# grantneale/kafka-lag-based-assignor

Hardware: AMD Instinct MI355X
Metric: partition-assignments/sec (whole node) (higher is better)
Workload: dtype int64

## Files before the change

kafka_lag_based_assignor_amd/csrc/la_api.hip:

```cpp
#include "la_ctx.h"

#include <dlfcn.h>

namespace {

constexpr int kMaxShards = 64;

struct HintSpender {
    la_ctx* ctx;
    explicit HintSpender(la_ctx* c) : ctx(c) {}
    ~HintSpender() { if (ctx) ctx->hints_set = false; }
    HintSpender(const HintSpender&) = delete;
    HintSpender& operator=(const HintSpender&) = delete;
};

struct RcclApi {
    void* handle = nullptr;
    int (*CommInitAll)(void** comms, int ndev, const int* devlist) = nullptr;
    int (*CommDestroy)(void* comm) = nullptr;
    int (*AllGather)(const void* send, void* recv, size_t count, int datatype, void* comm, hipStream_t stream) = nullptr;
    int (*GroupStart)() = nullptr;
    int (*GroupEnd)() = nullptr;
    const char* (*GetErrorString)(int) = nullptr;
    std::string why;
// ... 237 lines not shown
        g.out_pid = b->d_out_partition;
        g.out_rank = b->d_out_member_rank;
        g.out_total = b->d_out_total_lag;
        g.reset_latest = (b->reset_mode == LA_RESET_LATEST) ? 1 : 0;
        g.no_sample_sort = (b->flags & LA_FLAG_NO_SAMPLE_SORT) ? 1 : ((b->flags & LA_FLAG_SAMPLE_TIGHT) ? 2 : 0);
        g.sort_multi_kernel = (b->flags & LA_FLAG_SORT_MULTIKERNEL) ? 1 : 0;
        g.no_run_merge = (b->flags & LA_FLAG_NO_RUN_MERGE) ? 1 : 0;
        g.no_moved_sort = (b->flags & LA_FLAG_NO_MOVED_SORT) ? 1 : 0;
        const bool bounded_large = (b->flags & LA_FLAG_BOUNDS) && b->max_lag_hint >= 0 && b->max_partition_id_hint >= 0;
        g.max_lag_hint = bounded_large ? b->max_lag_hint : -1;
        g.max_id_hint = bounded_large ? b->max_partition_id_hint : -1;
        g.status = status;
        hipError_t e = hipSuccess;
        if (c > la::kLargeMaxConsumers) {
            if (int rc = flush()) return rc;
            if (argmin)
                return fail(ctx, LA_ESHAPE, "topic %lld has %lld consumers; LA_ALGO_ARGMIN (a test hook) holds at most %lld",
                            (long long)t, (long long)c, (long long)la::kLargeMaxConsumers);
            e = la::huge_topic_launch(ln.large, g, stream);
        } else if (argmin || p == 0 || (b->flags & LA_FLAG_SERIAL_LARGE)) {
            if (int rc = flush()) return rc;
            e = la::large_topic_launch(ln.large, g, argmin, stream);
        } else {
            if (group.size() >= kGroupTopics || (group_n > 0 && group_n + p > kGroupPartitions))
                if (int rc = flush()) return rc;
            group.push_back(g);
            group_n += p;
        }
        if (e != hipSuccess) return hip_fail(ctx, e, "large topic %lld: %s", (long long)t);
    }
    return flush();
}

}

int enqueue_batch(la_ctx* ctx, Lane& ln, const la_device_batch* b, hipStream_t stream, StagedBatch* staged) {
    uint32_t* const status = staged && staged->status ? staged->status : ln.d_status;
    const la::TileTail* const tail = staged ? staged->tail : nullptr;
    bool* const tail_done = staged ? &staged->tail_done : nullptr;
    if (b->n_topics < 0 || b->n_partitions < 0 || b->n_consumers < 0)
        return fail(ctx, LA_EINVAL, "negative size");
    if (b->n_topics == 0) return LA_OK;
    if (!b->d_part_off || !b->d_cons_off) return fail(ctx, LA_EINVAL, "null offsets");
    const bool wire_out = (b->flags & LA_FLAG_WIRE_OUT) != 0;
    if (b->n_partitions > 0 && !wire_out && (!b->d_out_partition || !b->d_out_member_rank)) return fail(ctx, LA_EINVAL, "null outputs");
    if (wire_out) {
        if (!b->d_out_wire || (b->wire_elem_bytes != 2 && b->wire_elem_bytes != 4) ||
            !la::wire_format_valid(b->wire_elem_bytes, b->wire_id_bits))
            return fail(ctx, LA_EINVAL, "LA_FLAG_WIRE_OUT: d_out_wire and a 2- or 4-byte wire format are required");
        if (b->algo != LA_ALGO_AUTO || (b->flags & LA_FLAG_RAGGED) ||
            !la::wave_tile_fits(b->max_partitions_per_topic, b->max_consumers_per_topic) || b->n_partitions >= ((int64_t)1 << 29) ||
            b->n_consumers >= ((int64_t)1 << 30) || (b->flags & LA_FLAG_INDEX64) || !(b->flags & LA_FLAG_BOUNDS) ||
            !la::wave_tile_always_packs(b->max_partitions_per_topic, b->max_consumers_per_topic, b->max_lag_hint,
                                        b->max_partition_id_hint))
            return fail(ctx, LA_EINVAL, "LA_FLAG_WIRE_OUT needs a batch of tile-sized topics (shape hint within 1024 x 64, no LA_FLAG_RAGGED), "
                                        "LA_FLAG_BOUNDS that prove every tile packs, and fewer than 2^29 partitions: run this batch "
                                        "without the flag and pack the results with la_pack_results_on");
    }
    if (b->n_partitions > 0 && (!b->d_partition_id || (!b->d_lag && (!b->d_end_off || !b->d_committed_off))))
        return fail(ctx, LA_EINVAL, "null per-partition input");
    if (b->n_consumers > 0 && !b->d_cons_rank) return fail(ctx, LA_EINVAL, "null cons_rank");
    if (!b->d_lag && b->reset_mode != LA_RESET_LATEST && !b->d_begin_off && b->n_partitions > 0)
        return fail(ctx, LA_EINVAL, "begin_off is required unless reset_mode is LA_RESET_LATEST");
    if (b->algo != LA_ALGO_AUTO && b->algo != LA_ALGO_ROUNDS && b->algo != LA_ALGO_ARGMIN && b->algo != LA_ALGO_ROUNDS_WIDE)
        return fail(ctx, LA_EINVAL, "unknown algo %d", b->algo);

    la::TileArgs a{};
    a.n_topics = b->n_topics;
    a.part_off = b->d_part_off;
    a.pid = b->d_partition_id;
    a.begin = b->d_begin_off;
    a.end = b->d_end_off;
    a.committed = b->d_committed_off;
    a.lag = b->d_lag;
    a.cons_off = b->d_cons_off;
    a.cons_rank = b->d_cons_rank;
    a.out_pid = b->d_out_partition;
    a.out_rank = b->d_out_member_rank;
    a.out_total = b->d_out_total_lag;
    a.status = status;
    a.reset_latest = (b->reset_mode == LA_RESET_LATEST) ? 1 : 0;
    a.n_total = b->n_partitions;
    a.flags = b->flags & (LA_FLAG_INDEX64 | LA_FLAG_DEFER_WIDE);
    if (getenv("LA_TILE_ALWAYS_STAGE2")) a.flags |= la::kTileAlwaysStage2;
    if (wire_out) {
        a.flags |= la::kTileWireOut;
        a.out_wire = b->d_out_wire;
        a.wire_bytes = b->wire_elem_bytes;
        a.wire_id_bits = b->wire_id_bits;
    }
    a.topic_list = nullptr;
    a.k_total = b->n_consumers;
    if (int rc = reserve(ctx, ln.defer, la::wave_tile_defer_bytes(b->n_topics))) return rc;
    a.defer_list = (int32_t*)ln.defer.p;
    const bool argmin = (b->algo == LA_ALGO_ARGMIN);
    const int tile_mode = argmin ? 2 : (b->algo == LA_ALGO_ROUNDS_WIDE ? 1 : 0);

    hipStreamCaptureStatus capture = hipStreamCaptureStatusNone;
    if (tile_mode == 0) LA_HIP(ctx, hipStreamIsCapturing(stream, &capture));
    hipError_t counter_err = hipSuccess;
    const bool bounded = tile_mode == 0 && (b->flags & LA_FLAG_BOUNDS) && b->max_lag_hint >= 0 && b->max_partition_id_hint >= 0;
    auto proven = [&](int64_t mp, int64_t mc) {
        return bounded && la::wave_tile_always_packs(mp, mc, b->max_lag_hint, b->max_partition_id_hint);
    };
    auto next_counters = [&](la::TileArgs& t) {
        int32_t* pair = (int32_t*)(ln.d_status + 16);
        if (t.flags & la::kTileNoDefer) {
            t.defer_count = pair + (ln.launches & 1u);
            t.defer_count_next = pair + ((ln.launches + 1u) & 1u);
            return;
        }
        if (capture != hipStreamCaptureStatusNone) {
            t.defer_count = pair + 2;
            t.defer_count_next = pair + 3;
            const hipError_t e = hipMemsetAsync(pair + 2, 0, sizeof(int32_t), stream);
            if (e != hipSuccess) counter_err = e;
            return;
        }
        t.defer_count = pair + (ln.launches & 1u);
        t.defer_count_next = pair + ((ln.launches + 1u) & 1u);
        if (tile_mode == 0) ++ln.launches;
    };
    if (b->n_partitions == 0) {
        if (b->d_out_total_lag && b->n_consumers > 0)
            LA_HIP(ctx, hipMemsetAsync(b->d_out_total_lag, 0, (size_t)b->n_consumers * sizeof(int64_t), stream));
        return LA_OK;
    }
    ln.large.prof.armed = (b->flags & LA_FLAG_PROFILE) != 0;
    if (ln.large.prof.armed) ln.large.prof.recorded = false;
    const bool have_host = b->h_part_off && b->h_cons_off;
    const bool fits_hint = la::wave_tile_fits(b->max_partitions_per_topic, b->max_consumers_per_topic);
    if (fits_hint && !(have_host && (b->flags & LA_FLAG_RAGGED) && tile_mode == 0)) {
        if (proven(b->max_partitions_per_topic, b->max_consumers_per_topic)) a.flags |= la::kTileNoDefer;
        next_counters(a);
        LA_HIP(ctx, counter_err);
        if (tail && tile_mode == 0) a.tail = *tail;
        LA_HIP(ctx, la::wave_tile_launch(a, b->max_partitions_per_topic, b->max_consumers_per_topic, tile_mode, stream,
                                         tail_done));
        return LA_OK;
    }
    la_device_batch with_host;
    if (!have_host) {
        hipStreamCaptureStatus cap = hipStreamCaptureStatusNone;
        LA_HIP(ctx, hipStreamIsCapturing(stream, &cap));
        if (cap != hipStreamCaptureStatusNone)
            return fail(ctx, LA_EINVAL, "shape hint exceeds one wave tile: h_part_off and h_cons_off are required "
                                        "while the stream is being captured");
        const size_t words = (size_t)b->n_topics + 1;
        ln.host_offsets.resize(2 * words);
        LA_HIP(ctx, hipMemcpyAsync(ln.host_offsets.data(), b->d_part_off, words * 8, hipMemcpyDeviceToHost, stream));
        LA_HIP(ctx, hipMemcpyAsync(ln.host_offsets.data() + words, b->d_cons_off, words * 8, hipMemcpyDeviceToHost, stream));
        LA_HIP(ctx, hipStreamSynchronize(stream));
        with_host = *b;
        with_host.h_part_off = ln.host_offsets.data();
        with_host.h_cons_off = ln.host_offsets.data() + words;
        b = &with_host;
    }

    const bool use_block = !argmin && b->algo != LA_ALGO_ROUNDS_WIDE;
    BatchPlan plan;
    if (int rc = plan_batch(ctx, ln, b, tile_mode, use_block, &plan)) return rc;
    const int32_t* d_lists = nullptr;
    if (int rc = stage_topic_lists(ctx, ln, plan, b->n_topics, stream, &d_lists)) return rc;
    if (plan.classed) {
        for (int k = 0; k < kTileClasses; ++k) {
            if (plan.tile[k].n == 0) continue;
            la::TileArgs run = a;
// ... 1443 lines not shown
```

kafka_lag_based_assignor_amd/csrc/la_kernels.h:

```cpp
#pragma once
#include <hip/hip_runtime.h>
#include <stdint.h>

#include "la_launch.h"

namespace la {

constexpr uint32_t kStatusShape = 1u;
constexpr uint32_t kStatusUnsorted = 2u;
constexpr uint32_t kStatusInternal = 4u;

constexpr uint32_t kStatusOrder = 8u;

constexpr uint32_t kStatusWire = 16u;

constexpr uint32_t kStatusSparse = 32u;

constexpr uint32_t kStatusBounds = 64u;

constexpr uint32_t kStatusLoads = 128u;

constexpr uint32_t kStatusMoves = 256u;

constexpr uint32_t kStatusCoop = 2 * kStatusMoves;

constexpr uint32_t kStatusSticky = 2 * kStatusCoop;

constexpr uint32_t kStatusBits[] = {kStatusShape, kStatusUnsorted, kStatusInternal, kStatusOrder,  kStatusWire,  kStatusSparse,
                                    kStatusBounds, kStatusLoads,   kStatusMoves,    kStatusCoop,   kStatusSticky};
constexpr bool status_bits_distinct() {
    uint32_t seen = 0;
    for (uint32_t b : kStatusBits) {
        if (b == 0 || (b & (b - 1)) != 0 || (seen & b) != 0) return false;
        seen |= b;
    }
    return true;
}
static_assert(status_bits_distinct(), "every status bit is one bit of its own");

constexpr int32_t kTileNoDefer = 8;
constexpr int32_t kTileWireOut = 16;
constexpr int32_t kTileSkipOversize = 4;
constexpr int32_t kTileAlwaysStage2 = 32;

constexpr int64_t kTileMaxPartitions = 1024;
constexpr int64_t kTileMaxConsumers = 64;
constexpr int64_t kLargeMaxConsumers = 8192;

struct TileTail {
    int32_t enabled;
    int32_t n_members;
    int32_t n;
    int32_t pad_;
    int64_t n_topics;
    const int64_t* part_off;
    const int32_t* out_pid;
    const int32_t* out_rank;
    int64_t* member_off;
    int32_t* grouped_topic;
    int32_t* grouped_partition;
    uint32_t* counter;
    uint32_t* fin_flag;
};

struct TileArgs {
    int64_t n_topics;
    int64_t n_total;
    int64_t k_total;
    const int64_t* part_off;
    const int32_t* pid;
    const int64_t* begin;
    const int64_t* end;
    const int64_t* committed;
    const int64_t* lag;
    const int64_t* cons_off;
    const int32_t* cons_rank;
    int32_t* out_pid;
    int32_t* out_rank;
    int64_t* out_total;
    uint32_t* status;
    int32_t reset_latest;
    int32_t flags;
    const int32_t* topic_list;
    int32_t* defer_count;
    int32_t* defer_count_next;
    int32_t* defer_list;
    TileTail tail;
    void* out_wire;
    int32_t wire_bytes, wire_id_bits;
};

inline size_t wave_tile_defer_bytes(int64_t n_topics) { return (size_t)(n_topics > 0 ? n_topics : 1) * sizeof(int32_t); }

inline bool wave_tile_fits(int64_t max_p, int64_t max_c) {
    return max_p <= kTileMaxPartitions && max_c <= kTileMaxConsumers;
}
void wave_tile_pick(int64_t max_p, int64_t max_c, int* L, int* E);
bool wave_tile_always_packs(int64_t max_p, int64_t max_c, int64_t max_lag, int64_t max_id);
hipError_t wave_tile_launch(TileArgs a, int64_t max_p, int64_t max_c, int mode, hipStream_t stream, bool* tail_done = nullptr);

hipError_t lag_launch(int64_t n, const int64_t* begin, const int64_t* end, const int64_t* committed,
                      bool reset_latest, int64_t* out_lag, hipStream_t stream);

hipError_t sparse_begin_launch(int64_t m, const int64_t* idx, const int64_t* val, int64_t base, int64_t lo, int64_t hi,
                               int64_t* begin, uint32_t* status, hipStream_t stream);

hipError_t finish_status_launch(const uint32_t* d_status, uint32_t* h_flag, hipStream_t stream);
hipError_t wake_launch(hipStream_t stream);

hipError_t check_consumers_launch(int64_t n_topics, const int64_t* cons_off, const int32_t* cons_rank,
                                  uint32_t* status, hipStream_t stream);

constexpr int64_t kBlockMaxPartitions = 8192;
constexpr int64_t kBlockMaxConsumers = 2048;
constexpr int64_t kBlockWidePartitions = 16384;
constexpr int64_t kBlockWideConsumers = 1024;
constexpr int kBlockClasses = 5;

struct BlockArgs {
    const int64_t* part_off;
    const int64_t* cons_off;
    const int32_t* list;
    int32_t n_list;
    int32_t inline_list[8];
    const int32_t* pid;
    const int64_t* begin;
    const int64_t* end;
    const int64_t* committed;
    const int64_t* lag;
    const int32_t* cons_rank;
    int32_t* out_pid;
    int32_t* out_rank;
    int64_t* out_total;
    uint32_t* status;
    int32_t reset_latest;
    int32_t np_cap, nc_cap;
    int32_t dense_ids;
    int32_t key32_greedy;
    int32_t radix_sort;
};

inline bool block_fits(int64_t p, int64_t c) {
    return (p <= kBlockMaxPartitions && c <= kBlockMaxConsumers) || (p <= kBlockWidePartitions && c <= kBlockWideConsumers);
}
inline int block_class(int64_t p, int64_t c) {
    if (p <= 512 && c <= 256) return 0;
    if (p <= 2048 && c <= 256) return 1;
    if (p <= 4096 && c <= 1024) return 2;
    if (p <= kBlockMaxPartitions) return 3;
    return 4;
}
hipError_t block_launch(BlockArgs a, int cls, hipStream_t stream);

struct LargeProfile {
    hipEvent_t ev[4] = {};
    bool armed = false;
    bool recorded = false;
    int64_t n = 0;
};

struct LargeScratch {
    void* buf = nullptr;
    size_t cap = 0;
    LargeProfile prof;
    struct Stage {
        void* h = nullptr;
        size_t cap = 0;
        hipEvent_t done = nullptr;
    } stage[2];
    unsigned stage_next = 0;
    void* d_items = nullptr;
    size_t d_items_cap = 0;
};

// ... 175 lines not shown
```

kafka_lag_based_assignor_amd/csrc/la_wave_tile_impl.h:

```cpp
#pragma once
#include "la_kernels.h"
#include "la_device.h"
#include "la_sort64.h"
#include "la_sort32.h"
#include "la_group_small.h"
#ifdef LA_LAB
#include <cstdio>
#include <cstdlib>
#endif

namespace la {

enum : int { kModeAuto = 0, kModeWide = 1, kModeArgmin = 2 };

#ifndef LA_ABLATE
#define LA_ABLATE 0
#endif
constexpr int kAblate = LA_ABLATE;
#ifndef LA_SKIP_SORTED_ROUNDS
#define LA_SKIP_SORTED_ROUNDS 1
#endif
constexpr bool kSkipSortedRounds = LA_SKIP_SORTED_ROUNDS != 0;
#ifndef LA_WPB
#define LA_WPB 4
#endif

template <int L, int E>
struct TileCfg {
    static constexpr int kGroupsPerWave = kWave / L;
    static constexpr int kWavesPerBlock = LA_WPB;
    static constexpr int kThreads = kWave * kWavesPerBlock;
    static constexpr int kTopicsPerBlock = kGroupsPerWave * kWavesPerBlock;
    static constexpr int kCap = L * E;
    static constexpr int kSlots = kCap + (kCap >> 3) + 1;
    static constexpr int kLog2Cap = (kCap <= 1) ? 0 : (31 - __builtin_clz(kCap - 1)) + 1;
};

__device__ __forceinline__ int slot_of(int s) { return s + (s >> 3); }

struct __attribute__((aligned(8))) I64x2 { int64_t x, y; };
struct __attribute__((aligned(4))) I32x2 { int32_t x, y; };

template <int L, int E>
__device__ __forceinline__ int load_index(int v, int gl) {
    if constexpr (E >= 2) return (v >> 1) * (2 * L) + 2 * gl + (v & 1);
    else return gl;
}

template <int E>
struct Raw {
    I64x2 en[(E + 1) / 2];
    I64x2 cm[(E + 1) / 2];
    I32x2 id[(E + 1) / 2];
};

template <typename IDX>
struct TopicDescT {
    IDX p0, c0;
    int P, C;
};
using TopicDesc = TopicDescT<int64_t>;

#ifndef LA_NT_LOADS
#define LA_NT_LOADS 1
#endif
template <typename V, typename T, typename IDX>
__device__ __forceinline__ V load_at(const T* base, IDX idx) {
    const V* p;
    if constexpr (sizeof(IDX) == 4)
        p = reinterpret_cast<const V*>(reinterpret_cast<const char*>(base) + (uint32_t)(idx * (uint32_t)sizeof(T)));
    else
        p = reinterpret_cast<const V*>(base + idx);
#if LA_NT_LOADS
    if constexpr (sizeof(V) == 16) {
        typedef long long LL2 __attribute__((ext_vector_type(2), aligned(8)));
        const LL2 v = __builtin_nontemporal_load(reinterpret_cast<const LL2*>(p));
        V out;
        __builtin_memcpy(&out, &v, 16);
        return out;
    } else if constexpr (sizeof(V) == 8) {
        typedef int I2 __attribute__((ext_vector_type(2), aligned(4)));
        const I2 v = __builtin_nontemporal_load(reinterpret_cast<const I2*>(p));
        V out;
        __builtin_memcpy(&out, &v, 8);
        return out;
    } else {
        return *p;
    }
#else
    return *p;
#endif
}

template <int L, int E, bool FULL = false, typename D>
__device__ __forceinline__ auto clamped_index(const TileArgs& a, const D& d, int v, int gl) {
    using IDX = decltype(d.p0);
    const IDX g = d.p0 + (IDX)load_index<L, E>(v, gl);
    if constexpr (FULL) return g;
    const IDX hi = (IDX)(a.n_total - (E >= 2 ? 2 : 1));
    return g < hi ? g : hi;
}

template <int L, int E, bool FULL = false, typename D>
__device__ __forceinline__ void issue_loads(const TileArgs& a, const D& d, int gl, Raw<E>& raw) {
    if constexpr (kAblate == 2) return;
    constexpr int NP = (E + 1) / 2;
    const int64_t* src_en = a.lag ? a.lag : a.end;
    if (!a.lag) {
#pragma unroll
        for (int k = 0; k < NP; ++k) {
            const auto g = clamped_index<L, E, FULL>(a, d, 2 * k, gl);
            if constexpr (E >= 2) raw.cm[k] = load_at<I64x2>(a.committed, g);
            else { raw.cm[k].x = load_at<int64_t>(a.committed, g); raw.cm[k].y = 0; }
        }
    } else {
#pragma unroll
        for (int k = 0; k < NP; ++k) raw.cm[k].x = raw.cm[k].y = 0;
    }
#pragma unroll
    for (int k = 0; k < NP; ++k) {
        const auto g = clamped_index<L, E, FULL>(a, d, 2 * k, gl);
        if constexpr (E >= 2) {
            raw.en[k] = load_at<I64x2>(src_en, g);
            raw.id[k] = load_at<I32x2>(a.pid, g);
        } else {
            raw.en[k].x = load_at<int64_t>(src_en, g); raw.en[k].y = 0;
            raw.id[k].x = load_at<int32_t>(a.pid, g); raw.id[k].y = 0;
        }
    }
}

template <int L, int E>
__device__ __forceinline__ bool second_stage_needed(const TileArgs& a) {
    return !a.lag && !a.reset_latest && a.begin;
}

template <int L, int E, bool FULL = false, typename D>
__device__ __forceinline__ void issue_begin_loads(const TileArgs& a, const D& d, int gl, Raw<E>& raw) {
    if constexpr (kAblate == 2) return;
    constexpr int NP = (E + 1) / 2;
    if (!second_stage_needed<L, E>(a)) return;
    {
        bool any = false;
#pragma unroll
        for (int k = 0; k < NP; ++k) any |= (raw.cm[k].x < 0) | (E >= 2 && raw.cm[k].y < 0);
        if (__builtin_amdgcn_ballot_w64(any) == 0 && !(a.flags & kTileAlwaysStage2)) return;
    }
#pragma unroll
    for (int k = 0; k < NP; ++k) {
        const auto g = clamped_index<L, E, FULL>(a, d, 2 * k, gl);
        using G = decltype(g);
        const bool nx = raw.cm[k].x < 0;
        if constexpr (E >= 2) {
            const bool ny = raw.cm[k].y < 0;
            const I64x2 bv = load_at<I64x2>(a.begin, (nx | ny) ? g : (G)0);
            raw.cm[k].x = nx ? bv.x : raw.cm[k].x;
            raw.cm[k].y = ny ? bv.y : raw.cm[k].y;
        } else {
            const int64_t vx = a.begin[nx ? g : (G)0];
            raw.cm[k].x = nx ? vx : raw.cm[k].x;
        }
    }
}

template <int L, int E, bool FULL = false, typename D>
__device__ __forceinline__ void finish_lags(const TileArgs& a, const D& d, int gl, const Raw<E>& raw,
                                            int64_t (&lag)[E], int32_t (&pid)[E]) {
    const bool latest = a.reset_latest != 0;
    if constexpr (kAblate == 2) {
#pragma unroll
        for (int v = 0; v < E; ++v) {
            const uint32_t h = ((uint32_t)d.p0 + (uint32_t)(v * L + gl)) * 2654435761u;
            lag[v] = (int64_t)(h >> 2) + a.reset_latest;
            pid[v] = (int32_t)((v * L + gl) * 77 + 13) & (L * E - 1);
        }
        return;
    }
    constexpr int NP = (E + 1) / 2;
    const bool cm_is_next = second_stage_needed<L, E>(a);
    auto lag_of = [&](int64_t en, int64_t cm) -> int64_t {
        if (a.lag) return en;
        if (cm_is_next) { const int64_t dlt = (int64_t)((uint64_t)en - (uint64_t)cm); return dlt > 0 ? dlt : 0; }
        return partition_lag(0, en, cm, latest);
    };
#pragma unroll
    for (int k = 0; k < NP; ++k) {
        const int e = load_index<L, E>(2 * k, gl);
        const bool shifted = !FULL && (E >= 2) && (d.p0 + (decltype(d.p0))e == (decltype(d.p0))(a.n_total - 1));
        const int64_t en_x = shifted ? raw.en[k].y : raw.en[k].x;
        const int64_t cm_x = shifted ? raw.cm[k].y : raw.cm[k].x;
        pid[2 * k] = shifted ? raw.id[k].y : raw.id[k].x;
        lag[2 * k] = lag_of(en_x, cm_x);
        if constexpr (E >= 2) {
            pid[2 * k + 1] = raw.id[k].y;
            lag[2 * k + 1] = lag_of(raw.en[k].y, raw.cm[k].y);
        }
    }
    if constexpr (FULL) return;
#pragma unroll
    for (int v = 0; v < E; ++v) {
        const bool valid = load_index<L, E>(v, gl) < d.P;
        lag[v] = valid ? lag[v] : 0;
        pid[v] = valid ? pid[v] : 0;
    }
}

template <int L, int E, bool FULL = false>
__device__ __forceinline__ void pack_records(int P, int gl, const int64_t (&lag)[E], const int32_t (&pid)[E], int sh,
                                             uint64_t lag_max, P64 (&rec)[E]) {
#pragma unroll
    for (int v = 0; v < E; ++v) {
        const int e = load_index<L, E>(v, gl);
        rec[v] = p64_from((FULL || e < P) ? (((lag_max - (uint64_t)lag[v]) << sh) | (uint32_t)pid[v]) : ~0ull);
    }
}

template <int L, int E, bool FULL = false>
__device__ __forceinline__ void sort_into_slice(uint64_t* slice, int gl, P64 (&rec)[E], int lbw, int sh) {
    using Cfg = TileCfg<L, E>;
    if constexpr (kAblate == 1 || kAblate == 4) {
#pragma unroll
        for (int r = 0; r < E; ++r) slice[slot_of(gl * E + r)] = p64_value(rec[r]);
        return;
    }
#ifdef LA_TILE_SORT64
    bitonic_sort_tile_p64<L, E>(rec);
#pragma unroll
    for (int r = 0; r < E; ++r) slice[slot_of(gl * E + r)] = p64_value(rec[r]);
    return;
#endif
    const bool by_id = sh <= Cfg::kLog2Cap;
    const int idx_bits = by_id ? sh : Cfg::kLog2Cap;
    const uint32_t idx_mask = (1u << idx_bits) - 1;
    const int top_bits = by_id ? lbw : lbw + sh;
    const int keep = 31 - idx_bits;
    const int drop = (by_id ? sh : 0) + (top_bits > keep ? top_bits - keep : 0);
    uint32_t key[E];
    if (by_id && drop == sh) {
#pragma unroll
        for (int v = 0; v < E; ++v) key[v] = (!FULL && rec[v].hi == 0xFFFFFFFFu) ? 0xFFFFFFFFu : rec[v].lo;
        bitonic_sort_tile_u32<L, E>(key);
#pragma unroll
        for (int r = 0; r < E; ++r)
            slice[slot_of(gl * E + r)] = (!FULL && key[r] == 0xFFFFFFFFu) ? ~0ull : (uint64_t)key[r];
        return;
    }
#pragma unroll
    for (int v = 0; v < E; ++v) {
        const uint64_t r = p64_value(rec[v]);
        const bool valid = FULL || r != ~0ull;
        const uint32_t idx = by_id ? ((uint32_t)r & idx_mask) : (uint32_t)load_index<L, E>(v, gl);
        if (valid) slice[slot_of((int)idx)] = r;
        key[v] = valid ? (((uint32_t)(r >> drop) << idx_bits) | idx) : 0xFFFFFFFFu;
    }
    wave_lds_fence();
    bitonic_sort_tile_u32<L, E>(key);

    P64 got[E];
#pragma unroll
    for (int r = 0; r < E; ++r) {
        const uint64_t x = slice[slot_of((int)(key[r] & idx_mask))];
        got[r] = p64_from((!FULL && key[r] == 0xFFFFFFFFu) ? ~0ull : x);
    }
    bool bad = false;
#pragma unroll
    for (int r = 0; r + 1 < E; ++r) {
        const uint64_t x = p64_value(got[r]), y = p64_value(got[r + 1]);
        bad |= (x >= y) && (FULL || y != ~0ull);
    }
    {
        const uint64_t x = p64_value(got[E - 1]);
        const uint64_t y = p64_of_next_lane(got[0]);
        bad |= (gl != L - 1) && (x >= y) && (FULL || y != ~0ull);
    }
    wave_lds_fence();
    if (__builtin_amdgcn_ballot_w64(bad) != 0) {
        bitonic_sort_tile_p64<L, E>(rec);
#pragma unroll
// ... 235 lines not shown
    }
    wave_lds_fence();

    if (a.out_total && bin.tb < (uint32_t)C)
        a.out_total[c0 + bin.tb] = (int64_t)(total ^ kTotalBias);
#pragma unroll
    for (int v = 0; v < E; ++v) {
        const int s = v * L + gl;
        if (s < P) {
            int32_t m = -1;
            if (C > 0) m = a.cons_rank[c0 + (uint32_t)slice[slot_of(s)]];
            a.out_rank[p0 + s] = m;
        }
    }
}

struct DescWords {
    int64_t p0, p1, c0, c1;
    bool exists;
};

template <int L, int E>
__device__ __forceinline__ DescWords fetch_desc(const TileArgs& a, int64_t t, int64_t n_tiles, int grp) {
    using Cfg = TileCfg<L, E>;
    const int64_t topic = t * Cfg::kGroupsPerWave + grp;
    DescWords w;
    w.exists = t < n_tiles && topic < a.n_topics;
    int64_t tc = w.exists ? topic : a.n_topics - 1;
    if (a.topic_list) tc = a.topic_list[tc];
    w.p0 = a.part_off[tc]; w.p1 = a.part_off[tc + 1];
    w.c0 = a.cons_off[tc]; w.c1 = a.cons_off[tc + 1];
    return w;
}

template <int L, int E>
__device__ __forceinline__ DescWords fetch_desc_uniform(const TileArgs& a, int64_t t, int grp) {
    constexpr int G = TileCfg<L, E>::kGroupsPerWave;
    typedef const int64_t __attribute__((address_space(4))) * ConstWords;
    const ConstWords po = (ConstWords)(uintptr_t)a.part_off + t * G;
    const ConstWords co = (ConstWords)(uintptr_t)a.cons_off + t * G;
    int64_t pw[G + 1], cw[G + 1];
#pragma unroll
    for (int k = 0; k <= G; ++k) { pw[k] = po[k]; cw[k] = co[k]; }
    DescWords w;
    w.exists = true;
    w.p0 = pw[0]; w.p1 = pw[1];
    w.c0 = cw[0]; w.c1 = cw[1];
#pragma unroll
    for (int g = 1; g < G; ++g) {
        const bool mine = grp >= g;
        w.p0 = mine ? pw[g] : w.p0; w.p1 = mine ? pw[g + 1] : w.p1;
        w.c0 = mine ? cw[g] : w.c0; w.c1 = mine ? cw[g + 1] : w.c1;
    }
    return w;
}

template <int L, int E, typename IDX = int64_t>
__device__ __forceinline__ TopicDescT<IDX> make_desc(const TileArgs& a, const DescWords& w, int gl) {
    using Cfg = TileCfg<L, E>;
    TopicDescT<IDX> d;
    d.p0 = (IDX)w.p0;
    d.c0 = (IDX)w.c0;
    const int64_t Pl = w.p1 - w.p0, Cl = w.c1 - w.c0;
    const bool bad = Pl > Cfg::kCap || Cl > L || Pl < 0 || Cl < 0;
    if (w.exists && bad && gl == 0 && !(a.flags & kTileSkipOversize)) atomicOr(a.status, kStatusShape);
    d.P = (w.exists && !bad) ? (int)Pl : 0;
    d.C = (w.exists && !bad) ? (int)Cl : 0;
    return d;
}

template <int L, int E, typename IDX = int64_t>
__device__ __forceinline__ TopicDescT<IDX> load_desc(const TileArgs& a, int64_t t, int64_t n_tiles, int grp, int gl) {
    return make_desc<L, E, IDX>(a, fetch_desc<L, E>(a, t, n_tiles, grp), gl);
}

template <int L, int E, typename IDX = int64_t>
__device__ __forceinline__ TopicDescT<IDX> load_desc_uniform(const TileArgs& a, int64_t t, int64_t n_tiles, int grp, int gl) {
    constexpr int G = TileCfg<L, E>::kGroupsPerWave;
    if (!a.topic_list && (t + 1) * G <= a.n_topics)
        return make_desc<L, E, IDX>(a, fetch_desc_uniform<L, E>(a, t, grp), gl);
    return make_desc<L, E, IDX>(a, fetch_desc<L, E>(a, t, n_tiles, grp), gl);
}

template <int L, int E, typename IDX, bool INLINE_WIDE, bool FULL, bool WIRE = false>
__device__ __forceinline__ void packed_tile(const TileArgs& a, const TopicDescT<IDX>& cur, uint64_t* slice, int32_t* rank_tab,
                                            int64_t tile, int gl, int lane) {
    using Cfg = TileCfg<L, E>;
    Raw<E> raw;
    issue_loads<L, E, FULL>(a, cur, gl, raw);
    int32_t my_rank = 0;
    if constexpr (kAblate != 2) {
        const IDX want = cur.c0 + (IDX)gl, last = (IDX)(a.k_total > 0 ? a.k_total - 1 : 0);
        if (a.k_total > 0) my_rank = load_at<int32_t>(a.cons_rank, want < last ? want : last);
    }
    issue_begin_loads<L, E, FULL>(a, cur, gl, raw);

    P64 rec[E];
    int sh, lbw;
    bool fits;
    uint64_t lag_max;
    int64_t lag[E];
    int32_t pid[E];
    {
        finish_lags<L, E, FULL>(a, cur, gl, raw, lag, pid);
        uint32_t id_or = 0;
        uint64_t lag_or = 0;
#pragma unroll
        for (int v = 0; v < E; ++v) { id_or |= (uint32_t)pid[v]; lag_or |= (uint64_t)lag[v]; }
        id_or = wave_or_u32_uniform(id_or);
        sh = 32 - __builtin_clz(id_or | 1u);
        lbw = bits_of_or_u64(wave_or_u32_uniform((uint32_t)(lag_or >> 32)), wave_or_u32_uniform((uint32_t)lag_or));
        int lim = 63 - sh;
        if (lim > 57 - Cfg::kLog2Cap) lim = 57 - Cfg::kLog2Cap;
        fits = sh < 32 && lbw <= lim;
        lag_max = lbw >= 64 ? ~0ull : (((uint64_t)1 << lbw) - 1);
        if (fits) pack_records<L, E, FULL>(cur.P, gl, lag, pid, sh, lag_max, rec);
    }
    if (fits) {
        sort_into_slice<L, E, FULL>(slice, gl, rec, lbw, sh);
        assign_packed<L, E, FULL, WIRE>(a, slice, rank_tab, cur.p0, cur.c0, cur.P, cur.C, gl, sh, lag_max, my_rank);
    } else if constexpr (INLINE_WIDE) {
        assign_wide<L, E, false>(a, slice, (int64_t)cur.p0, (int64_t)cur.c0, cur.P, cur.C, gl, lag, pid);
    } else if (lane == 0) {
        if (a.flags & kTileNoDefer) atomicOr(a.status, kStatusBounds);
        else a.defer_list[atomicAdd(a.defer_count, 1)] = (int32_t)tile;
    }
}

__device__ __forceinline__ void tile_tail(const TileTail& t, const uint32_t* status) {
    __shared__ uint32_t s_start[kTailGroupM];
    __shared__ int32_t s_in[7 * kSmallGroupN];
    __shared__ uint32_t s_wsum[LA_WPB];
    __shared__ uint32_t s_turn, s_last;
    __threadfence_system();
    __syncthreads();
    if (threadIdx.x == 0) {
        const uint32_t done = __hip_atomic_fetch_add(t.counter, 1u, __ATOMIC_ACQ_REL, __HIP_MEMORY_SCOPE_AGENT);
        s_last = done == gridDim.x - 1 ? 1u : 0u;
    }
    __syncthreads();
    if (!s_last) return;
    __builtin_amdgcn_fence(__ATOMIC_ACQUIRE, "agent");
    if (threadIdx.x == 0) __hip_atomic_store(t.counter, 0u, __ATOMIC_RELAXED, __HIP_MEMORY_SCOPE_AGENT);
    if (t.member_off)
        group_small_body_staged<kWave * LA_WPB, kTailGroupM>(t.n, t.n_members, t.n_topics, t.part_off, t.out_pid, t.out_rank,
                                                             t.member_off, t.grouped_topic, t.grouped_partition, nullptr, s_start,
                                                             s_wsum, &s_turn, s_in, s_in + kSmallGroupN, s_in + 2 * kSmallGroupN,
                                                             s_in + 3 * kSmallGroupN, s_in + 4 * kSmallGroupN,
                                                             reinterpret_cast<uint32_t*>(s_in + 5 * kSmallGroupN),
                                                             reinterpret_cast<uint32_t*>(s_in + 6 * kSmallGroupN));
    __threadfence_system();
    __syncthreads();
    if (threadIdx.x == 0) {
        const uint32_t st = __hip_atomic_load(status, __ATOMIC_RELAXED, __HIP_MEMORY_SCOPE_AGENT);
        __hip_atomic_store(t.fin_flag, 0x80000000u | st, __ATOMIC_RELEASE, __HIP_MEMORY_SCOPE_SYSTEM);
    }
}

#ifdef LA_WPE
#define LA_WPE_ATTR __attribute__((amdgpu_waves_per_eu(LA_WPE, LA_WPE)))
#else
#define LA_WPE_ATTR
#endif
template <int L, int E, typename IDX, bool INLINE_WIDE, bool WIRE = false>
__global__ __launch_bounds__(256) LA_WPE_ATTR void wave_tile_packed_kernel(TileArgs a) {
    using Cfg = TileCfg<L, E>;
    __shared__ uint64_t lds[Cfg::kTopicsPerBlock * Cfg::kSlots];
    __shared__ int32_t rank_lds[Cfg::kTopicsPerBlock * L];

    const int lane = threadIdx.x & (kWave - 1);
    const int wave = __builtin_amdgcn_readfirstlane((int)(threadIdx.x >> 6));
    const int gl = lane & (L - 1);
    const int grp = lane / L;
    uint64_t* slice = lds + (wave * Cfg::kGroupsPerWave + grp) * Cfg::kSlots;
    int32_t* rank_tab = rank_lds + (wave * Cfg::kGroupsPerWave + grp) * L;

    const int64_t n_tiles = (a.n_topics + Cfg::kGroupsPerWave - 1) / Cfg::kGroupsPerWave;
    const int64_t tile = (int64_t)blockIdx.x * Cfg::kWavesPerBlock + wave;
    if constexpr (INLINE_WIDE) {
        if (blockIdx.x == 0 && threadIdx.x == 0) *a.defer_count_next = 0;
        if (tile < n_tiles) {
            const TopicDescT<IDX> cur = load_desc_uniform<L, E, IDX>(a, tile, n_tiles, grp, gl);
            packed_tile<L, E, IDX, true, false>(a, cur, slice, rank_tab, tile, gl, lane);
        }
        if (a.tail.enabled) tile_tail(a.tail, a.status);
        return;
    }
    if (tile >= n_tiles) return;
    const TopicDescT<IDX> cur = load_desc_uniform<L, E, IDX>(a, tile, n_tiles, grp, gl);
    if constexpr (!INLINE_WIDE) {
        if (__builtin_amdgcn_ballot_w64(cur.P != Cfg::kCap || (int64_t)cur.p0 + Cfg::kCap > a.n_total) == 0) {
            packed_tile<L, E, IDX, false, true, WIRE>(a, cur, slice, rank_tab, tile, gl, lane);
            return;
        }
    }
    packed_tile<L, E, IDX, INLINE_WIDE, false, WIRE>(a, cur, slice, rank_tab, tile, gl, lane);
}

template <int L, int E, bool ARGMIN>
__global__ __launch_bounds__(256) void wave_tile_wide_kernel(TileArgs a, int from_list) {
    using Cfg = TileCfg<L, E>;
    __shared__ uint64_t lds[Cfg::kTopicsPerBlock * Cfg::kSlots];

    const int lane = threadIdx.x & (kWave - 1);
    const int wave = threadIdx.x >> 6;
    const int gl = lane & (L - 1);
    const int grp = lane / L;
    uint64_t* slice = lds + (wave * Cfg::kGroupsPerWave + grp) * Cfg::kSlots;

    const int64_t n_tiles = (a.n_topics + Cfg::kGroupsPerWave - 1) / Cfg::kGroupsPerWave;
    const int64_t n_waves = (int64_t)gridDim.x * Cfg::kWavesPerBlock;
    const int64_t count = from_list ? (int64_t)*a.defer_count : n_tiles;
    if (from_list && blockIdx.x == 0 && threadIdx.x == 0) *a.defer_count_next = 0;
    for (int64_t i = (int64_t)blockIdx.x * Cfg::kWavesPerBlock + wave; i < count; i += n_waves) {
        const int64_t tile = from_list ? (int64_t)a.defer_list[i] : i;
        const TopicDesc d = load_desc<L, E>(a, tile, n_tiles, grp, gl);
        Raw<E> raw;
        issue_loads<L, E>(a, d, gl, raw);
        issue_begin_loads<L, E>(a, d, gl, raw);
        int64_t lag[E];
        int32_t pid[E];
        finish_lags<L, E>(a, d, gl, raw, lag, pid);
        assign_wide<L, E, ARGMIN>(a, slice, d.p0, d.c0, d.P, d.C, gl, lag, pid);
        wave_lds_fence();
    }
}

template <typename K>
static hipError_t resident_blocks(K kernel, int threads, int* out) {
    int dev = 0, cus = 0, per_cu = 0;
    hipError_t e;
    if ((e = hipGetDevice(&dev)) != hipSuccess) return e;
    if ((e = hipDeviceGetAttribute(&cus, hipDeviceAttributeMultiprocessorCount, dev)) != hipSuccess) return e;
    if ((e = hipOccupancyMaxActiveBlocksPerMultiprocessor(&per_cu, kernel, threads, 0)) != hipSuccess) return e;
    if (per_cu < 1) per_cu = 1;
    *out = cus * per_cu;
    return hipSuccess;
}

template <int L, int E>
static hipError_t launch_one(const TileArgs& a_in, int mode, hipStream_t stream, bool* tail_done) {
    TileArgs a = a_in;
    const bool want_tail = a.tail.enabled != 0;
    a.tail.enabled = 0;
    using Cfg = TileCfg<L, E>;
    const int64_t blocks = (a.n_topics + Cfg::kTopicsPerBlock - 1) / Cfg::kTopicsPerBlock;
    if (blocks <= 0) return hipSuccess;
    struct Res { std::atomic<int> inl{0}, wide{0}, argmin{0}; };
    static Res s_res[33];
    hipError_t e;
    int dev = 0;
    if ((e = hipGetDevice(&dev)) != hipSuccess) return e;
    const bool cached = dev >= 0 && dev < 32;
    Res& rs = s_res[cached ? dev : 32];
    std::atomic<int>&s_inline = rs.inl, &s_wide = rs.wide, &s_argmin = rs.argmin;
    int res_inline = cached ? s_inline.load(std::memory_order_acquire) : 0, res_wide = s_wide.load(std::memory_order_relaxed),
        res_argmin = s_argmin.load(std::memory_order_relaxed);
    if (res_inline == 0) {
        if ((e = resident_blocks(wave_tile_packed_kernel<L, E, uint32_t, true>, Cfg::kThreads, &res_inline)) != hipSuccess) return e;
        if ((e = resident_blocks(wave_tile_wide_kernel<L, E, false>, Cfg::kThreads, &res_wide)) != hipSuccess) return e;
        if ((e = resident_blocks(wave_tile_wide_kernel<L, E, true>, Cfg::kThreads, &res_argmin)) != hipSuccess) return e;
        if (cached) {
            s_wide.store(res_wide, std::memory_order_relaxed);
            s_argmin.store(res_argmin, std::memory_order_relaxed);
            s_inline.store(res_inline, std::memory_order_release);
        }
#ifdef LA_LAB
        printf("resident blocks: inline %d wide %d argmin %d (needed %lld)\n", res_inline, res_wide, res_argmin, (long long)blocks);
#endif
    }
    const dim3 b(Cfg::kThreads);
    auto grid = [&](int resident) { return dim3((unsigned)(blocks < resident ? blocks : resident)); };
    if (mode == kModeArgmin) {
        LA_LAUNCH((wave_tile_wide_kernel<L, E, true>), grid(res_argmin), b, 0, stream, a, 0);
    } else if (mode == kModeWide) {
        LA_LAUNCH((wave_tile_wide_kernel<L, E, false>), grid(res_wide), b, 0, stream, a, 0);
    } else {
        if (!a.defer_count || !a.defer_count_next || !a.defer_list) return hipErrorInvalidValue;
        const bool idx32 = a.n_total < ((int64_t)1 << 29) && a.k_total < ((int64_t)1 << 30) && !(a.flags & 1);
        if (idx32 && blocks <= res_inline && !(a.flags & 2) && !(a.flags & kTileWireOut)) {
            if (want_tail && tail_done) {
                a.tail.enabled = 1;
                *tail_done = true;
            }
            LA_LAUNCH((wave_tile_packed_kernel<L, E, uint32_t, true>), dim3((unsigned)blocks), b, 0, stream, a);
            return hipGetLastError();
        }
        if (a.flags & kTileWireOut) {
            if (!idx32 || !(a.flags & kTileNoDefer) || !a.out_wire) return hipErrorInvalidValue;
            LA_LAUNCH((wave_tile_packed_kernel<L, E, uint32_t, false, true>), dim3((unsigned)blocks), b, 0, stream, a);
            return hipGetLastError();
        }
        if (idx32)
            LA_LAUNCH((wave_tile_packed_kernel<L, E, uint32_t, false>), dim3((unsigned)blocks), b, 0, stream, a);
        else
            LA_LAUNCH((wave_tile_packed_kernel<L, E, int64_t, false>), dim3((unsigned)blocks), b, 0, stream, a);
        if (a.flags & kTileNoDefer) return hipGetLastError();
#ifdef LA_LAB
        if (getenv("LA_NO_WIDE")) return hipGetLastError();
#endif
        LA_LAUNCH((wave_tile_wide_kernel<L, E, false>), grid(res_wide), b, 0, stream, a, 1);
    }
    return hipGetLastError();
}

template <int L>
static inline hipError_t launch_l(int e, const TileArgs& a, int mode, hipStream_t stream, bool* tail_done) {
    switch (e) {
        case 1: return launch_one<L, 1>(a, mode, stream, tail_done);
        case 2: return launch_one<L, 2>(a, mode, stream, tail_done);
        case 4: return launch_one<L, 4>(a, mode, stream, tail_done);
        case 8: return launch_one<L, 8>(a, mode, stream, tail_done);
        default: return launch_one<L, 16>(a, mode, stream, tail_done);
    }
}

}
```

Measured before the change: 195.6 billion.

## Specialize packed tile kernel on lag mode and tune waves per EU

Adds a compile-time lag-mode template parameter (lags given, with begin offsets, without begin) to the packed tile kernel. The idx32 non-inline launches pick the matching instantiation at runtime, so per-element branches on lag/begin/reset fold away, and sign tests use only the high 32-bit word. It also sets amdgpu_waves_per_eu for the E=8 with-begin variant to steer register allocation, and caches a getenv lookup in a static. The cost is more kernel instantiations, and the forced wave count could cause spills.

```diff
diff --git a/kafka_lag_based_assignor_amd/csrc/la_api.hip b/kafka_lag_based_assignor_amd/csrc/la_api.hip
--- a/kafka_lag_based_assignor_amd/csrc/la_api.hip
+++ b/kafka_lag_based_assignor_amd/csrc/la_api.hip
@@ -343,7 +343,8 @@
     a.reset_latest = (b->reset_mode == LA_RESET_LATEST) ? 1 : 0;
     a.n_total = b->n_partitions;
     a.flags = b->flags & (LA_FLAG_INDEX64 | LA_FLAG_DEFER_WIDE);
-    if (getenv("LA_TILE_ALWAYS_STAGE2")) a.flags |= la::kTileAlwaysStage2;
+    static const bool always_stage2 = getenv("LA_TILE_ALWAYS_STAGE2") != nullptr;
+    if (always_stage2) a.flags |= la::kTileAlwaysStage2;
     if (wire_out) {
         a.flags |= la::kTileWireOut;
         a.out_wire = b->d_out_wire;
diff --git a/kafka_lag_based_assignor_amd/csrc/la_kernels.h b/kafka_lag_based_assignor_amd/csrc/la_kernels.h
--- a/kafka_lag_based_assignor_amd/csrc/la_kernels.h
+++ b/kafka_lag_based_assignor_amd/csrc/la_kernels.h
@@ -42,6 +42,13 @@
 constexpr int32_t kTileWireOut = 16;
 constexpr int32_t kTileSkipOversize = 4;
 constexpr int32_t kTileAlwaysStage2 = 32;
+
+enum : int {
+    kLagRuntime = 0,
+    kLagGiven = 1,
+    kLagNoBegin = 2,
+    kLagWithBegin = 3,
+};
 
 constexpr int64_t kTileMaxPartitions = 1024;
 constexpr int64_t kTileMaxConsumers = 64;
@@ -90,6 +97,10 @@
     int32_t wire_bytes, wire_id_bits;
 };
 
+inline int tile_lag_mode(const TileArgs& a) {
+    return a.lag ? kLagGiven : ((!a.reset_latest && a.begin) ? kLagWithBegin : kLagNoBegin);
+}
+
 inline size_t wave_tile_defer_bytes(int64_t n_topics) { return (size_t)(n_topics > 0 ? n_topics : 1) * sizeof(int32_t); }
 
 inline bool wave_tile_fits(int64_t max_p, int64_t max_c) {
diff --git a/kafka_lag_based_assignor_amd/csrc/la_wave_tile_impl.h b/kafka_lag_based_assignor_amd/csrc/la_wave_tile_impl.h
--- a/kafka_lag_based_assignor_amd/csrc/la_wave_tile_impl.h
+++ b/kafka_lag_based_assignor_amd/csrc/la_wave_tile_impl.h
@@ -101,12 +101,19 @@
     return g < hi ? g : hi;
 }
 
-template <int L, int E, bool FULL = false, typename D>
+template <int LM>
+__device__ __forceinline__ bool lags_given(const TileArgs& a) {
+    if constexpr (LM == kLagRuntime) return a.lag != nullptr;
+    else return LM == kLagGiven;
+}
+
+template <int L, int E, bool FULL = false, int LM = kLagRuntime, typename D>
 __device__ __forceinline__ void issue_loads(const TileArgs& a, const D& d, int gl, Raw<E>& raw) {
     if constexpr (kAblate == 2) return;
     constexpr int NP = (E + 1) / 2;
-    const int64_t* src_en = a.lag ? a.lag : a.end;
-    if (!a.lag) {
+    const bool given = lags_given<LM>(a);
+    const int64_t* src_en = given ? a.lag : a.end;
+    if (!given) {
 #pragma unroll
         for (int k = 0; k < NP; ++k) {
             const auto g = clamped_index<L, E, FULL>(a, d, 2 * k, gl);
@@ -130,43 +137,60 @@
     }
 }
 
-template <int L, int E>
+template <int LM>
 __device__ __forceinline__ bool second_stage_needed(const TileArgs& a) {
-    return !a.lag && !a.reset_latest && a.begin;
-}
-
-template <int L, int E, bool FULL = false, typename D>
+    if constexpr (LM == kLagRuntime) return !a.lag && !a.reset_latest && a.begin;
+    else return LM == kLagWithBegin;
+}
+
+__device__ __forceinline__ int32_t hi_word(int64_t v) { return (int32_t)((uint64_t)v >> 32); }
+
+template <int L, int E, bool FULL = false, int LM = kLagRuntime, typename D>
 __device__ __forceinline__ void issue_begin_loads(const TileArgs& a, const D& d, int gl, Raw<E>& raw) {
     if constexpr (kAblate == 2) return;
     constexpr int NP = (E + 1) / 2;
-    if (!second_stage_needed<L, E>(a)) return;
+    if (!second_stage_needed<LM>(a)) return;
     {
-        bool any = false;
-#pragma unroll
-        for (int k = 0; k < NP; ++k) any |= (raw.cm[k].x < 0) | (E >= 2 && raw.cm[k].y < 0);
-        if (__builtin_amdgcn_ballot_w64(any) == 0 && !(a.flags & kTileAlwaysStage2)) return;
+        int32_t none = 0;
+#pragma unroll
+        for (int k = 0; k < NP; ++k) none |= hi_word(raw.cm[k].x) | (E >= 2 ? hi_word(raw.cm[k].y) : 0);
+        if (__builtin_amdgcn_ballot_w64(none < 0) == 0 && !(a.flags & kTileAlwaysStage2)) return;
     }
 #pragma unroll
     for (int k = 0; k < NP; ++k) {
         const auto g = clamped_index<L, E, FULL>(a, d, 2 * k, gl);
         using G = decltype(g);
-        const bool nx = raw.cm[k].x < 0;
+        const int32_t hx = hi_word(raw.cm[k].x);
         if constexpr (E >= 2) {
-            const bool ny = raw.cm[k].y < 0;
-            const I64x2 bv = load_at<I64x2>(a.begin, (nx | ny) ? g : (G)0);
-            raw.cm[k].x = nx ? bv.x : raw.cm[k].x;
-            raw.cm[k].y = ny ? bv.y : raw.cm[k].y;
+            const int32_t hy = hi_word(raw.cm[k].y);
+            const I64x2 bv = load_at<I64x2>(a.begin, (hx | hy) < 0 ? g : (G)0);
+            raw.cm[k].x = hx < 0 ? bv.x : raw.cm[k].x;
+            raw.cm[k].y = hy < 0 ? bv.y : raw.cm[k].y;
         } else {
-            const int64_t vx = a.begin[nx ? g : (G)0];
-            raw.cm[k].x = nx ? vx : raw.cm[k].x;
-        }
-    }
-}
-
-template <int L, int E, bool FULL = false, typename D>
+            const int64_t vx = a.begin[hx < 0 ? g : (G)0];
+            raw.cm[k].x = hx < 0 ? vx : raw.cm[k].x;
+        }
+    }
+}
+
+template <int LM>
+__device__ __forceinline__ void lag_pair(const TileArgs& a, int64_t en_x, int64_t cm_x, int64_t en_y, int64_t cm_y,
+                                         int64_t& lag_x, int64_t& lag_y) {
+    if (lags_given<LM>(a)) { lag_x = en_x; lag_y = en_y; return; }
+    int64_t nx = cm_x, ny = cm_y;
+    if (!second_stage_needed<LM>(a)) {
+        const bool latest = a.reset_latest != 0;
+        nx = hi_word(cm_x) < 0 ? (latest ? en_x : 0) : cm_x;
+        ny = hi_word(cm_y) < 0 ? (latest ? en_y : 0) : cm_y;
+    }
+    const int64_t dx = (int64_t)((uint64_t)en_x - (uint64_t)nx), dy = (int64_t)((uint64_t)en_y - (uint64_t)ny);
+    lag_x = hi_word(dx) < 0 ? 0 : dx;
+    lag_y = hi_word(dy) < 0 ? 0 : dy;
+}
+
+template <int L, int E, bool FULL = false, int LM = kLagRuntime, typename D>
 __device__ __forceinline__ void finish_lags(const TileArgs& a, const D& d, int gl, const Raw<E>& raw,
                                             int64_t (&lag)[E], int32_t (&pid)[E]) {
-    const bool latest = a.reset_latest != 0;
     if constexpr (kAblate == 2) {
 #pragma unroll
         for (int v = 0; v < E; ++v) {
@@ -177,12 +201,6 @@
         return;
     }
     constexpr int NP = (E + 1) / 2;
-    const bool cm_is_next = second_stage_needed<L, E>(a);
-    auto lag_of = [&](int64_t en, int64_t cm) -> int64_t {
-        if (a.lag) return en;
-        if (cm_is_next) { const int64_t dlt = (int64_t)((uint64_t)en - (uint64_t)cm); return dlt > 0 ? dlt : 0; }
-        return partition_lag(0, en, cm, latest);
-    };
 #pragma unroll
     for (int k = 0; k < NP; ++k) {
         const int e = load_index<L, E>(2 * k, gl);
@@ -190,10 +208,11 @@
         const int64_t en_x = shifted ? raw.en[k].y : raw.en[k].x;
         const int64_t cm_x = shifted ? raw.cm[k].y : raw.cm[k].x;
         pid[2 * k] = shifted ? raw.id[k].y : raw.id[k].x;
-        lag[2 * k] = lag_of(en_x, cm_x);
+        int64_t lag_y;
+        lag_pair<LM>(a, en_x, cm_x, raw.en[k].y, raw.cm[k].y, lag[2 * k], lag_y);
         if constexpr (E >= 2) {
             pid[2 * k + 1] = raw.id[k].y;
-            lag[2 * k + 1] = lag_of(raw.en[k].y, raw.cm[k].y);
+            lag[2 * k + 1] = lag_y;
         }
     }
     if constexpr (FULL) return;
@@ -595,18 +614,18 @@
     return make_desc<L, E, IDX>(a, fetch_desc<L, E>(a, t, n_tiles, grp), gl);
 }
 
-template <int L, int E, typename IDX, bool INLINE_WIDE, bool FULL, bool WIRE = false>
+template <int L, int E, typename IDX, bool INLINE_WIDE, bool FULL, bool WIRE = false, int LM = kLagRuntime>
 __device__ __forceinline__ void packed_tile(const TileArgs& a, const TopicDescT<IDX>& cur, uint64_t* slice, int32_t* rank_tab,
                                             int64_t tile, int gl, int lane) {
     using Cfg = TileCfg<L, E>;
     Raw<E> raw;
-    issue_loads<L, E, FULL>(a, cur, gl, raw);
+    issue_loads<L, E, FULL, LM>(a, cur, gl, raw);
     int32_t my_rank = 0;
     if constexpr (kAblate != 2) {
         const IDX want = cur.c0 + (IDX)gl, last = (IDX)(a.k_total > 0 ? a.k_total - 1 : 0);
         if (a.k_total > 0) my_rank = load_at<int32_t>(a.cons_rank, want < last ? want : last);
     }
-    issue_begin_loads<L, E, FULL>(a, cur, gl, raw);
+    issue_begin_loads<L, E, FULL, LM>(a, cur, gl, raw);
 
     P64 rec[E];
     int sh, lbw;
@@ -615,7 +634,7 @@
     int64_t lag[E];
     int32_t pid[E];
     {
-        finish_lags<L, E, FULL>(a, cur, gl, raw, lag, pid);
+        finish_lags<L, E, FULL, LM>(a, cur, gl, raw, lag, pid);
         uint32_t id_or = 0;
         uint64_t lag_or = 0;
 #pragma unroll
@@ -673,9 +692,13 @@
 #ifdef LA_WPE
 #define LA_WPE_ATTR __attribute__((amdgpu_waves_per_eu(LA_WPE, LA_WPE)))
 #else
-#define LA_WPE_ATTR
-#endif
-template <int L, int E, typename IDX, bool INLINE_WIDE, bool WIRE = false>
+template <int L, int E, bool INLINE_WIDE, int LM>
+constexpr int tile_waves() {
+    return (!INLINE_WIDE && LM == kLagWithBegin && E == 8) ? (L == 64 ? 7 : 6) : 0;
+}
+#define LA_WPE_ATTR __attribute__((amdgpu_waves_per_eu(tile_waves<L, E, INLINE_WIDE, LM>(), tile_waves<L, E, INLINE_WIDE, LM>())))
+#endif
+template <int L, int E, typename IDX, bool INLINE_WIDE, bool WIRE = false, int LM = kLagRuntime>
 __global__ __launch_bounds__(256) LA_WPE_ATTR void wave_tile_packed_kernel(TileArgs a) {
     using Cfg = TileCfg<L, E>;
     __shared__ uint64_t lds[Cfg::kTopicsPerBlock * Cfg::kSlots];
@@ -703,11 +726,11 @@
     const TopicDescT<IDX> cur = load_desc_uniform<L, E, IDX>(a, tile, n_tiles, grp, gl);
     if constexpr (!INLINE_WIDE) {
         if (__builtin_amdgcn_ballot_w64(cur.P != Cfg::kCap || (int64_t)cur.p0 + Cfg::kCap > a.n_total) == 0) {
-            packed_tile<L, E, IDX, false, true, WIRE>(a, cur, slice, rank_tab, tile, gl, lane);
+            packed_tile<L, E, IDX, false, true, WIRE, LM>(a, cur, slice, rank_tab, tile, gl, lane);
             return;
         }
     }
-    packed_tile<L, E, IDX, INLINE_WIDE, false, WIRE>(a, cur, slice, rank_tab, tile, gl, lane);
+    packed_tile<L, E, IDX, INLINE_WIDE, false, WIRE, LM>(a, cur, slice, rank_tab, tile, gl, lane);
 }
 
 template <int L, int E, bool ARGMIN>
@@ -749,6 +772,15 @@
     if (per_cu < 1) per_cu = 1;
     *out = cus * per_cu;
     return hipSuccess;
+}
+
+template <int L, int E, bool WIRE>
+static void launch_lean(const TileArgs& a, dim3 grid, dim3 block, hipStream_t stream) {
+    switch (tile_lag_mode(a)) {
+        case kLagGiven: LA_LAUNCH((wave_tile_packed_kernel<L, E, uint32_t, false, WIRE, kLagGiven>), grid, block, 0, stream, a); break;
+        case kLagWithBegin: LA_LAUNCH((wave_tile_packed_kernel<L, E, uint32_t, false, WIRE, kLagWithBegin>), grid, block, 0, stream, a); break;
+        default: LA_LAUNCH((wave_tile_packed_kernel<L, E, uint32_t, false, WIRE, kLagNoBegin>), grid, block, 0, stream, a); break;
+    }
 }
 
 template <int L, int E>
@@ -801,11 +833,11 @@
         }
         if (a.flags & kTileWireOut) {
             if (!idx32 || !(a.flags & kTileNoDefer) || !a.out_wire) return hipErrorInvalidValue;
-            LA_LAUNCH((wave_tile_packed_kernel<L, E, uint32_t, false, true>), dim3((unsigned)blocks), b, 0, stream, a);
+            launch_lean<L, E, true>(a, dim3((unsigned)blocks), b, stream);
             return hipGetLastError();
         }
         if (idx32)
-            LA_LAUNCH((wave_tile_packed_kernel<L, E, uint32_t, false>), dim3((unsigned)blocks), b, 0, stream, a);
+            launch_lean<L, E, false>(a, dim3((unsigned)blocks), b, stream);
         else
             LA_LAUNCH((wave_tile_packed_kernel<L, E, int64_t, false>), dim3((unsigned)blocks), b, 0, stream, a);
         if (a.flags & kTileNoDefer) return hipGetLastError();
```

Result: no change. 196.1 billion (median of 6 runs) (+0.3%).
